# JiaruiFeng/KP-GNN

Hardware: AMD Instinct MI355X
Metric: graphs/sec KP-GIN fwd+bwd, ZINC-12k K=8 L=8 h=104 (higher is better)
Workload: dtype f32; 1 GPU; ZINC-12k-shaped synthetic molecules, KPGINPlus K=8 L=8 h=104 kernel=spd geometric combine, fwd+bwd+Adam, L1 loss; global_batch=2048, nodes_per_batch=47450, khop_edges_per_batch=1018372, active_pairs_per_batch=1018372, parallelism=dp1, launch=hipGraph replay of fwd+bwd, batches=4 pre-staged batches cycled

## Files before the change

kp_gnn_amd/csrc/wgrad.hip:

```cpp
#include <cstdlib>
#include <type_traits>

#include "bf3.h"
#include "kpgnn_common.h"

namespace kpgnn {
namespace {

constexpr int kWgradBlocks = 512;

struct WgParams {
    int64_t N; int O, I;
    const float* dy; int64_t dys;
    const float* x; int64_t xs;
    const float* xm; const float* xi; const float* xg; const float* xb; int xrelu;
    float* slab;
    int64_t slab_row, slab_off;
};
struct WgPair { WgParams q[2]; };

template <int TI, int RG>
__device__ __forceinline__ void wgrad_problem(const WgParams p, float* lds) {
    const int lane = threadIdx.x & 63;
    const int nstrip = (int)(blockDim.x >> 6) / RG;
    const int wave = (int)(threadIdx.x >> 6) % nstrip, rg = (int)(threadIdx.x >> 6) / nstrip;
    const int kk = lane >> 5, c = lane & 31;
    const int o = wave * 32 + c;
    const int64_t vgrid = (int64_t)gridDim.x * RG, vb = (int64_t)blockIdx.x * RG + rg;
    const bool o_ok = o < p.O;
    f32x16 acc[TI];
#pragma unroll
    for (int t = 0; t < TI; ++t)
        for (int v = 0; v < 16; ++v) acc[t][v] = 0.f;
    float bsum = 0.f;
    float tm[TI], ts[TI], tg[TI], tb[TI];
    const bool tr = p.xm != nullptr;
    if (tr) {
#pragma unroll
        for (int t = 0; t < TI; ++t) {
            const int i = t * 32 + c;
            const bool ok = i < p.I;
            tm[t] = ok ? p.xm[i] : 0.f; ts[t] = ok ? p.xi[i] : 0.f; tg[t] = ok ? p.xg[i] : 0.f; tb[t] = ok ? p.xb[i] : 0.f;
        }
    }
    const int64_t pairs = (p.N + 1) / 2;
    constexpr int UN = 4;
    const int dyo = kk * (int)p.dys + (o_ok ? o : p.O - 1);
    int xo[TI];
#pragma unroll
    for (int t = 0; t < TI; ++t) xo[t] = kk * (int)p.xs + min(t * 32 + c, p.I - 1);
    for (int64_t pr = vb; pr < pairs; pr += vgrid * UN) {
        float a[UN], b[UN][TI];
        const bool full = 2 * (pr + (int64_t)(UN - 1) * vgrid) + 1 < p.N;
        if (full) {
#pragma unroll
            for (int u = 0; u < UN; ++u) {
                const int64_t r0 = 2 * (pr + (int64_t)u * vgrid);
                const float* dyr = p.dy + r0 * p.dys;
                const float* xr = p.x + r0 * p.xs;
                a[u] = dyr[dyo];
#pragma unroll
                for (int t = 0; t < TI; ++t) b[u][t] = xr[xo[t]];
            }
            if (tr) {
#pragma unroll
                for (int u = 0; u < UN; ++u)
#pragma unroll
                    for (int t = 0; t < TI; ++t) {
                        float v = fmaf((b[u][t] - tm[t]) * ts[t], tg[t], tb[t]);
                        if (p.xrelu) v = fmaxf(v, 0.f);
                        b[u][t] = v;
                    }
            }
        } else {
#pragma unroll
            for (int u = 0; u < UN; ++u) {
                const int64_t r = 2 * (pr + (int64_t)u * vgrid) + kk;
                const bool r_ok = r < p.N;
                a[u] = (r_ok && o_ok) ? p.dy[r * p.dys + o] : 0.f;
#pragma unroll
                for (int t = 0; t < TI; ++t) {
                    const int i = t * 32 + c;
                    b[u][t] = (r_ok && i < p.I) ? p.x[r * p.xs + i] : 0.f;
                }
            }
            if (tr) {
#pragma unroll
                for (int u = 0; u < UN; ++u) {
                    const bool r_ok = 2 * (pr + (int64_t)u * vgrid) + kk < p.N;
#pragma unroll
                    for (int t = 0; t < TI; ++t) {
                        float v = fmaf((b[u][t] - tm[t]) * ts[t], tg[t], tb[t]);
                        if (p.xrelu) v = fmaxf(v, 0.f);
                        b[u][t] = (r_ok && t * 32 + c < p.I) ? v : 0.f;
                    }
                }
            }
        }
#pragma unroll
        for (int u = 0; u < UN; ++u) {
            bsum += a[u];
#pragma unroll
            for (int t = 0; t < TI; ++t) acc[t] = __builtin_amdgcn_mfma_f32_32x32x2f32(a[u], b[u][t], acc[t], 0, 0, 0);
        }
    }
    bsum += __shfl_xor(bsum, 32);
    if (RG > 1) {
        float* sl = lds + (size_t)wave * (TI * 16 + 1) * 64 + lane;
        __syncthreads();
        if (rg == 1) {
#pragma unroll
            for (int t = 0; t < TI; ++t)
                for (int v = 0; v < 16; ++v) sl[(t * 16 + v) * 64] = acc[t][v];
            sl[TI * 16 * 64] = bsum;
        }
        __syncthreads();
        if (rg == 0) {
#pragma unroll
            for (int t = 0; t < TI; ++t)
                for (int v = 0; v < 16; ++v) acc[t][v] += sl[(t * 16 + v) * 64];
            bsum += sl[TI * 16 * 64];
        }
    }
    float* out = p.slab + (int64_t)blockIdx.x * p.slab_row + p.slab_off;
    if (rg == 0) {
#pragma unroll
    for (int t = 0; t < TI; ++t) {
        const int i = t * 32 + c;
        for (int v = 0; v < 16; ++v) {
            const int orow = wave * 32 + (v & 3) + 8 * (v >> 2) + 4 * kk;
            if (orow < p.O && i < p.I) out[(int64_t)orow * p.I + i] = acc[t][v];
        }
    }
    if (kk == 0 && o_ok) out[(int64_t)p.O * p.I + o] = bsum;
    }
}

template <int TI, int RG>
__global__ void __launch_bounds__(512)
wgrad_kernel(const WgPair pp, int nprob) {
    extern __shared__ __attribute__((aligned(16))) float wg_lds[];
    if (gridDim.y > 1) {
        if (blockIdx.y == 0) wgrad_problem<TI, RG>(pp.q[0], wg_lds);
        else wgrad_problem<TI, RG>(pp.q[1], wg_lds);
        return;
    }
    wgrad_problem<TI, RG>(pp.q[0], wg_lds);
    if (nprob > 1) wgrad_problem<TI, RG>(pp.q[1], wg_lds);
}

int wgrad_grid(int64_t N) {
    int64_t g = (N + 15) / 16;
    if (g > kWgradBlocks) g = kWgradBlocks;
    return (int)(g < 1 ? 1 : g);
}

int wgrad_check(const kpgnn_wgrad_desc* d, const char* who) {
    KPGNN_REQUIRE(d != nullptr, "%s: NULL descriptor", who);
    KPGNN_REQUIRE(d->N >= 1 && d->O >= 1 && d->I >= 1, "%s: bad N=%lld O=%d I=%d", who, (long long)d->N, d->O, d->I);
    if (d->O > 256 || d->I > 256) return fail(KPGNN_ELIMIT, "%s: O=%d, I=%d exceed 256", who, d->O, d->I);
    KPGNN_REQUIRE(d->dy && d->x && d->dw && d->dy_stride >= d->O && d->x_stride >= d->I, "%s: bad pointers/strides", who);
    KPGNN_REQUIRE(!d->x_mean || (d->x_invstd && d->x_gamma && d->x_beta), "%s: x transform needs mean, invstd, gamma, beta", who);
    return KPGNN_OK;
}

WgParams wgrad_params(const kpgnn_wgrad_desc* d, float* slab, int64_t slab_row, int64_t slab_off) {
    WgParams p;
    p.N = d->N; p.O = d->O; p.I = d->I; p.dy = d->dy; p.dys = d->dy_stride; p.x = d->x; p.xs = d->x_stride;
    p.xm = d->x_mean; p.xi = d->x_invstd; p.xg = d->x_gamma; p.xb = d->x_beta; p.xrelu = d->x_relu;
    p.slab = slab; p.slab_row = slab_row; p.slab_off = slab_off;
    return p;
}

int wgrad_groups(int O) { return O <= 128 ? 2 : 1; }

int wgrad_blocks(int64_t N, int O) {
    const int rg = wgrad_groups(O);
    return (wgrad_grid(N) + rg - 1) / rg;
}

int wgrad_launch(const WgPair& pp, int nprob, int O, int I, int grid, hipStream_t s) {
    const int waves = (O + 31) / 32, ti = (I + 31) / 32, rg = wgrad_groups(O);
    dim3 blk(waves * 64 * rg), gr(grid, (nprob > 1 && grid * rg <= 128) ? 2 : 1);
    const size_t lds = rg > 1 ? sizeof(float) * (size_t)waves * (ti * 16 + 1) * 64 : 0;
#define KP_WG(T) do { \
        if (rg > 1) { KPGNN_HIP_TRY(ensure_dynamic_lds((const void*)wgrad_kernel<T, 2>, lds)); \
                      hipLaunchKernelGGL((wgrad_kernel<T, 2>), gr, blk, lds, s, pp, nprob); } \
        else hipLaunchKernelGGL((wgrad_kernel<T, 1>), gr, blk, 0, s, pp, nprob); } while (0)
    switch (ti) {
        case 1: KP_WG(1); break;
        case 2: KP_WG(2); break;
        case 3: KP_WG(3); break;
        case 4: KP_WG(4); break;
        case 5: KP_WG(5); break;
        case 6: KP_WG(6); break;
        case 7: KP_WG(7); break;
        default: KP_WG(8); break;
    }
#undef KP_WG
    KPGNN_LAUNCH_CHECK("wgrad_kernel");
    return KPGNN_OK;
}

constexpr int kW2Rows = 32;
constexpr int kW2MaxProb = 16;

struct Wg2Prob {
    const float* dy; const float* x; const float* mask;
    const float* xm; const float* xi; const float* xg; const float* xb;
    int xrelu;
    int64_t dys, xs, out_off, bias_off;
};
struct Wg2Args {
    int64_t N; const int32_t* n_dyn;
    int O, I, nprob; int64_t ldw;
    float* slab; int64_t slab_row;
    Wg2Prob q[kW2MaxProb];
};

template <int TI>
__global__ void __launch_bounds__(256, 2)
wgrad2_kernel(const Wg2Args A) {
    extern __shared__ __attribute__((aligned(16))) float w2[];
    constexpr int R = kW2Rows;
    const int O = A.O, I = A.I;
    float* dyl = w2;
    float* xl = w2 + R * O;
    float* coef = xl + R * I;
    const int tid = threadIdx.x, wave = tid >> 6, lane = tid & 63;
    const int kk = lane >> 5, c = lane & 31;
    const int nprob = A.nprob;
    const int pi = (int)(blockIdx.x % nprob), slice = (int)(blockIdx.x / nprob), nslices = (int)(gridDim.x / nprob);
    Wg2Prob q = A.q[0];
#pragma unroll
    for (int i = 1; i < kW2MaxProb; ++i)
        if (pi == i) q = A.q[i];
    const int64_t N = A.n_dyn ? (int64_t)min((int64_t)*A.n_dyn, A.N) : A.N;
    const bool tr = q.xm != nullptr;
    if (tr)
        for (int i = tid; i < I; i += 256) { coef[i] = q.xm[i]; coef[I + i] = q.xi[i]; coef[2 * I + i] = q.xg[i]; coef[3 * I + i] = q.xb[i]; }
    const int o4 = O >> 2, i4 = I >> 2;
    int dy_row[4], dy_cg[4], x_row[TI], x_cg[TI];
#pragma unroll
    for (int j = 0; j < 4; ++j) { const int e = tid + 256 * j; dy_row[j] = e < R * o4 ? e / o4 : -1; dy_cg[j] = e % o4; }
#pragma unroll
    for (int j = 0; j < TI; ++j) { const int e = tid + 256 * j; x_row[j] = e < R * i4 ? e / i4 : -1; x_cg[j] = e % i4; }
    float4 pdy[4], pm[4], px[TI];
    const bool has_mask = q.mask != nullptr;
    const int64_t last = N - 1;
    auto issue = [&](int64_t ch) {
        const int64_t r0 = ch * R;
#pragma unroll
        for (int j = 0; j < 4; ++j) {
            const int64_t r = min(r0 + max(dy_row[j], 0), last);
            pdy[j] = *reinterpret_cast<const float4*>(q.dy + r * q.dys + 4 * dy_cg[j]);
            if (has_mask) pm[j] = *reinterpret_cast<const float4*>(q.mask + r * q.dys + 4 * dy_cg[j]);
        }
#pragma unroll
        for (int j = 0; j < TI; ++j) {
            const int64_t r = min(r0 + max(x_row[j], 0), last);
            px[j] = *reinterpret_cast<const float4*>(q.x + r * q.xs + 4 * x_cg[j]);
        }
    };
    auto commit = [&](int64_t ch) {
        const int64_t r0 = ch * R;
        const float4 zero = make_float4(0.f, 0.f, 0.f, 0.f);
#pragma unroll
        for (int j = 0; j < 4; ++j) {
            float4 v = pdy[j];
            if (has_mask) { v.x = pm[j].x > 0.f ? v.x : 0.f; v.y = pm[j].y > 0.f ? v.y : 0.f; v.z = pm[j].z > 0.f ? v.z : 0.f; v.w = pm[j].w > 0.f ? v.w : 0.f; }
            if (r0 + dy_row[j] >= N) v = zero;
            if (dy_row[j] >= 0) *reinterpret_cast<float4*>(dyl + dy_row[j] * O + 4 * dy_cg[j]) = v;
        }
#pragma unroll
        for (int j = 0; j < TI; ++j) {
            float4 v = px[j];
            if (tr) {
                const float4 m = *reinterpret_cast<const float4*>(coef + 4 * x_cg[j]), s = *reinterpret_cast<const float4*>(coef + I + 4 * x_cg[j]);
                const float4 g = *reinterpret_cast<const float4*>(coef + 2 * I + 4 * x_cg[j]), b = *reinterpret_cast<const float4*>(coef + 3 * I + 4 * x_cg[j]);
                v.x = fmaf((v.x - m.x) * s.x, g.x, b.x); v.y = fmaf((v.y - m.y) * s.y, g.y, b.y);
                v.z = fmaf((v.z - m.z) * s.z, g.z, b.z); v.w = fmaf((v.w - m.w) * s.w, g.w, b.w);
                if (q.xrelu) { v.x = fmaxf(v.x, 0.f); v.y = fmaxf(v.y, 0.f); v.z = fmaxf(v.z, 0.f); v.w = fmaxf(v.w, 0.f); }
            }
            if (r0 + x_row[j] >= N) v = zero;
            if (x_row[j] >= 0) *reinterpret_cast<float4*>(xl + x_row[j] * I + 4 * x_cg[j]) = v;
        }
    };
    f32x16 acc[TI];
#pragma unroll
    for (int t = 0; t < TI; ++t)
        for (int v = 0; v < 16; ++v) acc[t][v] = 0.f;
    float bsum = 0.f;
    const int o = wave * 32 + c;
    const bool o_ok = o < O;
    const float* ap = dyl + kk * O + (o_ok ? o : O - 1);
    const float* bp[TI];
#pragma unroll
    for (int t = 0; t < TI; ++t) bp[t] = xl + kk * I + min(t * 32 + c, I - 1);
    const int64_t chunks = (N + R - 1) / R;
    int64_t ch = slice;
    if (tr) __syncthreads();
    if (ch < chunks) { issue(ch); commit(ch); }
    __syncthreads();
    for (; ch < chunks; ch += nslices) {
        const int64_t nx = ch + nslices;
        const bool more = nx < chunks;
        if (more) issue(nx);
#pragma unroll
        for (int p2 = 0; p2 < R / 2; ++p2) {
            const float a = ap[2 * p2 * O];
            bsum += a;
#pragma unroll
            for (int t = 0; t < TI; ++t) acc[t] = __builtin_amdgcn_mfma_f32_32x32x2f32(a, bp[t][2 * p2 * I], acc[t], 0, 0, 0);
        }
        __syncthreads();
        if (more) commit(nx);
        __syncthreads();
    }
    bsum += __shfl_xor(bsum, 32);
    float* out = A.slab + (int64_t)slice * A.slab_row;
#pragma unroll
    for (int t = 0; t < TI; ++t) {
        const int i = t * 32 + c;
        for (int v = 0; v < 16; ++v) {
            const int orow = wave * 32 + (v & 3) + 8 * (v >> 2) + 4 * kk;
            if (orow < O && i < I) out[q.out_off + (int64_t)orow * A.ldw + i] = acc[t][v];
        }
    }
    if (q.bias_off >= 0 && kk == 0 && o_ok) out[q.bias_off + o] = bsum;
}

constexpr int kW3Pitch = 40;

constexpr int kW3Blocks = 256;

template <int TI, bool MASK>
__global__ void __launch_bounds__(512, 1)
wgrad3_kernel(const Wg2Args A) {
    extern __shared__ __attribute__((aligned(16))) float w2[];
    constexpr int R = kW2Rows, P = kW3Pitch;
    const int O = A.O, I = A.I;
    const int bufsz = 3 * (O + I) * P;
    __bf16* pl = reinterpret_cast<__bf16*>(w2);
    float* coef = reinterpret_cast<float*>(pl + 2 * bufsz);
    const int tid = threadIdx.x, lane = tid & 63;
    const int wave = __builtin_amdgcn_readfirstlane(tid >> 6);
    const int kg = lane >> 5, c = lane & 31;
    const int nprob = A.nprob;
    const int pi = (int)(blockIdx.x % nprob), slice = (int)(blockIdx.x / nprob), nslices = (int)(gridDim.x / nprob);
    Wg2Prob q = A.q[0];
#pragma unroll
    for (int i = 1; i < kW2MaxProb; ++i)
        if (pi == i) q = A.q[i];
    const int64_t N = A.n_dyn ? (int64_t)min((int64_t)*A.n_dyn, A.N) : A.N;
    const bool tr = q.xm != nullptr;
    if (tr)
        for (int i = tid; i < I; i += 512) { coef[i] = q.xm[i]; coef[I + i] = q.xi[i]; coef[2 * I + i] = q.xg[i]; coef[3 * I + i] = q.xb[i]; }
    const int64_t chunks = (N + R - 1) / R;
    const int64_t mine = slice < chunks ? (chunks - slice + nslices - 1) / nslices : 0;
    const bool producer = wave >= 4;
    const bool is_x = wave >= 6;
    const int ncg = (is_x ? I : O) >> 2;
    const int task = tid & 127;
    const bool owner = producer && task < 4 * ncg;
    const int g = owner ? task & 3 : 0, cg = owner ? task >> 2 : 0;
    const float* src = is_x ? q.x : q.dy;
    const int64_t sstride = is_x ? q.xs : q.dys;
    const uint32_t sbytes = (uint32_t)sstride * 4u;
    const bool xform = tr && is_x;
    const int64_t last = N - 1;
    bf3_f2 bs01 = {0.f, 0.f}, bs23 = {0.f, 0.f};
    auto produce = [&](auto mask_c) {
        constexpr bool M = decltype(mask_c)::value;
        float4 pv0[8], pm0[8], pv1[8], pm1[8];
        auto issue = [&](int64_t k, float4 (&pv)[8], float4 (&pm)[8]) {
            const int64_t c0 = (slice + min(k, mine - 1) * nslices) * R;
            const float* cp = src + c0 * sstride;
            const float* mp = M ? q.mask + c0 * sstride : nullptr;
            const int lim = (int)min((int64_t)R, N - c0) - 1;
#pragma unroll
            for (int j = 0; j < 8; ++j) {
                const uint32_t off = __umul24((uint32_t)min(8 * g + j, lim), sbytes) + 16u * (uint32_t)cg;
                pv[j] = *reinterpret_cast<const float4*>(reinterpret_cast<const char*>(cp) + off);
                if (M) pm[j] = *reinterpret_cast<const float4*>(reinterpret_cast<const char*>(mp) + off);
            }
        };
        auto commit = [&](int64_t k, float4 (&pv)[8], float4 (&pm)[8]) {
            const int64_t c0 = (slice + min(k, mine - 1) * nslices) * R;
            if (M) {
    #pragma unroll
                for (int j = 0; j < 8; ++j) {
                    pv[j].x = pm[j].x > 0.f ? pv[j].x : 0.f; pv[j].y = pm[j].y > 0.f ? pv[j].y : 0.f;
                    pv[j].z = pm[j].z > 0.f ? pv[j].z : 0.f; pv[j].w = pm[j].w > 0.f ? pv[j].w : 0.f;
                }
            }
            if (xform) {
                const float4 m4 = *reinterpret_cast<const float4*>(coef + 4 * cg), s4 = *reinterpret_cast<const float4*>(coef + I + 4 * cg);
                const float4 g4 = *reinterpret_cast<const float4*>(coef + 2 * I + 4 * cg), b4 = *reinterpret_cast<const float4*>(coef + 3 * I + 4 * cg);
    #pragma unroll
                for (int j = 0; j < 8; ++j) {
                    float4 v = pv[j];
                    v.x = fmaf((v.x - m4.x) * s4.x, g4.x, b4.x); v.y = fmaf((v.y - m4.y) * s4.y, g4.y, b4.y);
                    v.z = fmaf((v.z - m4.z) * s4.z, g4.z, b4.z); v.w = fmaf((v.w - m4.w) * s4.w, g4.w, b4.w);
                    if (q.xrelu) { v.x = fmaxf(v.x, 0.f); v.y = fmaxf(v.y, 0.f); v.z = fmaxf(v.z, 0.f); v.w = fmaxf(v.w, 0.f); }
                    pv[j] = v;
                }
            }
            if (c0 + R > N) {
    #pragma unroll
                for (int j = 0; j < 8; ++j)
                    if (c0 + 8 * g + j >= N) pv[j] = make_float4(0.f, 0.f, 0.f, 0.f);
            }
            if (!is_x && k < mine) {
    #pragma unroll
                for (int j = 0; j < 8; ++j) { bs01 += bf3_f2{pv[j].x, pv[j].y}; bs23 += bf3_f2{pv[j].z, pv[j].w}; }
            }
            if (owner) {
                __bf16* base = pl + (k & 1) * bufsz + (is_x ? 3 * O * P : 0) + 8 * g;
                const int cols = is_x ? I : O;
    #pragma unroll
                for (int e2 = 0; e2 < 2; ++e2) {
                    bf3_u2 h[8], m[8], l[8];
#pragma unroll
                    for (int j = 0; j < 8; ++j)
                        bf3_split2(e2 == 0 ? bf3_f2{pv[j].x, pv[j].y} : bf3_f2{pv[j].z, pv[j].w}, h[j], m[j], l[j]);
                    __bf16* col = base + (4 * cg + 2 * e2) * P;
                    *reinterpret_cast<uint4*>(col) = make_uint4(bf3_pack(h[0].x, h[1].x), bf3_pack(h[2].x, h[3].x), bf3_pack(h[4].x, h[5].x), bf3_pack(h[6].x, h[7].x));
                    *reinterpret_cast<uint4*>(col + P) = make_uint4(bf3_pack(h[0].y, h[1].y), bf3_pack(h[2].y, h[3].y), bf3_pack(h[4].y, h[5].y), bf3_pack(h[6].y, h[7].y));
                    *reinterpret_cast<uint4*>(col + cols * P) = make_uint4(bf3_pack(m[0].x, m[1].x), bf3_pack(m[2].x, m[3].x), bf3_pack(m[4].x, m[5].x), bf3_pack(m[6].x, m[7].x));
                    *reinterpret_cast<uint4*>(col + cols * P + P) = make_uint4(bf3_pack(m[0].y, m[1].y), bf3_pack(m[2].y, m[3].y), bf3_pack(m[4].y, m[5].y), bf3_pack(m[6].y, m[7].y));
                    *reinterpret_cast<uint4*>(col + 2 * cols * P) = make_uint4(bf3_pack(l[0].x, l[1].x), bf3_pack(l[2].x, l[3].x), bf3_pack(l[4].x, l[5].x), bf3_pack(l[6].x, l[7].x));
                    *reinterpret_cast<uint4*>(col + 2 * cols * P + P) = make_uint4(bf3_pack(l[0].y, l[1].y), bf3_pack(l[2].y, l[3].y), bf3_pack(l[4].y, l[5].y), bf3_pack(l[6].y, l[7].y));
                }
            }
        };
        __builtin_amdgcn_s_setprio(2);
        if (mine > 0) {
            issue(0, pv0, pm0);
            issue(1, pv1, pm1);
            commit(0, pv0, pm0);
            issue(2, pv0, pm0);
        }
        __syncthreads();
        for (int64_t k = 0; k < mine; k += 2) {
            commit(k + 1, pv1, pm1);
            issue(k + 3, pv1, pm1);
            __syncthreads();
            commit(k + 2, pv0, pm0);
            issue(k + 4, pv0, pm0);
            __syncthreads();
        }
    };
    f32x16 acc[TI];
#pragma unroll
    for (int t = 0; t < TI; ++t)
        for (int v = 0; v < 16; ++v) acc[t][v] = 0.f;
    const int o = wave * 32 + c;
    const bool strip = !producer && wave * 32 < O;
    const int aoff = min(o, O - 1) * P + 8 * kg;
    int boff[TI];
#pragma unroll
    for (int t = 0; t < TI; ++t) boff[t] = 3 * O * P + min(t * 32 + c, I - 1) * P + 8 * kg;
    auto ld8 = [&](const __bf16* ptr) { return __builtin_bit_cast(bf3_x8, *reinterpret_cast<const uint4*>(ptr)); };
    auto multiply = [&](int64_t k) {
        const __bf16* bf = pl + (k & 1) * bufsz;
#pragma unroll
        for (int ks = 0; ks < R / 16; ++ks) {
            const bf3_x8 ah = ld8(bf + aoff + 16 * ks), am = ld8(bf + aoff + O * P + 16 * ks), al = ld8(bf + aoff + 2 * O * P + 16 * ks);
            bf3_x8 bh[TI], bm[TI], bl[TI];
#pragma unroll
            for (int t = 0; t < TI; ++t) {
                bh[t] = ld8(bf + boff[t] + 16 * ks); bm[t] = ld8(bf + boff[t] + I * P + 16 * ks); bl[t] = ld8(bf + boff[t] + 2 * I * P + 16 * ks);
            }
#pragma unroll
            for (int t = 0; t < TI; ++t) acc[t] = __builtin_amdgcn_mfma_f32_32x32x16_bf16(al, bh[t], acc[t], 0, 0, 0);
#pragma unroll
            for (int t = 0; t < TI; ++t) acc[t] = __builtin_amdgcn_mfma_f32_32x32x16_bf16(ah, bl[t], acc[t], 0, 0, 0);
#pragma unroll
            for (int t = 0; t < TI; ++t) acc[t] = __builtin_amdgcn_mfma_f32_32x32x16_bf16(am, bm[t], acc[t], 0, 0, 0);
#pragma unroll
            for (int t = 0; t < TI; ++t) acc[t] = __builtin_amdgcn_mfma_f32_32x32x16_bf16(am, bh[t], acc[t], 0, 0, 0);
#pragma unroll
            for (int t = 0; t < TI; ++t) acc[t] = __builtin_amdgcn_mfma_f32_32x32x16_bf16(ah, bm[t], acc[t], 0, 0, 0);
#pragma unroll
            for (int t = 0; t < TI; ++t) acc[t] = __builtin_amdgcn_mfma_f32_32x32x16_bf16(ah, bh[t], acc[t], 0, 0, 0);
        }
    };
    if (tr) __syncthreads();
    float* out = A.slab + (int64_t)slice * A.slab_row;
    if (producer) {
        if (MASK && !is_x) produce(std::true_type{});
        else produce(std::false_type{});
    } else {
        __syncthreads();
        for (int64_t k = 0; k < mine; k += 2) {
            if (strip) multiply(k);

            __syncthreads();

            if (strip && k + 1 < mine) multiply(k + 1);

            __syncthreads();
        }
        if (strip) {
#pragma unroll
            for (int t = 0; t < TI; ++t) {
                const int i = t * 32 + c;
                for (int v = 0; v < 16; ++v) {
                    const int orow = wave * 32 + (v & 3) + 8 * (v >> 2) + 4 * kg;
                    if (orow < O && i < I) out[q.out_off + (int64_t)orow * A.ldw + i] = acc[t][v];
                }
            }
        }
    }
    if (q.bias_off >= 0) {
        if (owner && !is_x) *reinterpret_cast<float4*>(coef + g * O + 4 * cg) = make_float4(bs01.x, bs01.y, bs23.x, bs23.y);
        __syncthreads();
        if (tid < O) out[q.bias_off + tid] = (coef[tid] + coef[O + tid]) + (coef[2 * O + tid] + coef[3 * O + tid]);
    }
}

bool wgrad3_ok(const Wg2Args& A) {
    for (int i = 1; i < A.nprob; ++i)
        if ((A.q[i].mask != nullptr) != (A.q[0].mask != nullptr)) return false;
    for (int i = 0; i < A.nprob; ++i)
        if (A.q[i].dys >= (1 << 22) || A.q[i].xs >= (1 << 22)) return false;
    return A.O <= 128 && A.I <= 128;
}
size_t wgrad3_lds(const Wg2Args& A) {
    const int m = A.O > A.I ? A.O : A.I;
    return (size_t)2 * 2 * 3 * (A.O + A.I) * kW3Pitch + sizeof(float) * 4 * (size_t)m;
}

bool wgrad2_ok(const kpgnn_wgrad_desc* d, const float* x) {
    auto al = [](const void* q) { return (((uintptr_t)q) & 15) == 0; };
    return d->O % 4 == 0 && d->I % 4 == 0 && d->O <= 128 && d->I <= 256 && d->dy_stride % 4 == 0 && d->x_stride % 4 == 0 &&
           al(d->dy) && al(x) && (!d->dy_mask || al(d->dy_mask));
}

Wg2Prob wgrad2_prob(const kpgnn_wgrad_desc* d, const float* x, int64_t out_off, int64_t bias_off) {
    Wg2Prob q;
    q.dy = d->dy; q.x = x; q.mask = d->dy_mask; q.xm = d->x_mean; q.xi = d->x_invstd; q.xg = d->x_gamma; q.xb = d->x_beta;
    q.xrelu = d->x_relu; q.dys = d->dy_stride; q.xs = d->x_stride; q.out_off = out_off; q.bias_off = bias_off;
    return q;
}

int wgrad2_slices(int64_t N, int nprob, int blocks) {
    const int64_t chunks = (N + kW2Rows - 1) / kW2Rows;
    int64_t s = blocks / nprob;
    if (s > chunks) s = chunks;
    return (int)(s < 1 ? 1 : s);
}

int wgrad2_launch(Wg2Args& A, int math, int* nslices, hipStream_t s) {
    const int ti = (A.I + 31) / 32;
    if (math != KPGNN_MATH_F32 && wgrad3_ok(A)) {
        *nslices = wgrad2_slices(A.N, A.nprob, kW3Blocks);
        dim3 gr3((unsigned)(*nslices * A.nprob)), blk3(512);
        const size_t lds3 = wgrad3_lds(A);
        const bool mask = A.q[0].mask != nullptr;
#define KP_W3(T) do { if (mask) { KPGNN_HIP_TRY(ensure_dynamic_lds((const void*)wgrad3_kernel<T, true>, lds3)); \
                                  hipLaunchKernelGGL((wgrad3_kernel<T, true>), gr3, blk3, lds3, s, A); } \
                      else { KPGNN_HIP_TRY(ensure_dynamic_lds((const void*)wgrad3_kernel<T, false>, lds3)); \
                             hipLaunchKernelGGL((wgrad3_kernel<T, false>), gr3, blk3, lds3, s, A); } } while (0)
        switch (ti) {
            case 1: KP_W3(1); break;
            case 2: KP_W3(2); break;
            case 3: KP_W3(3); break;
            default: KP_W3(4); break;
        }
#undef KP_W3
        KPGNN_LAUNCH_CHECK("wgrad3_kernel");
        return KPGNN_OK;
    }
    *nslices = wgrad2_slices(A.N, A.nprob, kWgradBlocks);
    dim3 gr((unsigned)(*nslices * A.nprob)), blk(256);
    const size_t lds = sizeof(float) * ((size_t)kW2Rows * (A.O + A.I) + 4 * (size_t)A.I);
#define KP_W2(T) hipLaunchKernelGGL((wgrad2_kernel<T>), gr, blk, lds, s, A)
    switch (ti) {
        case 1: KP_W2(1); break;
        case 2: KP_W2(2); break;
        case 3: KP_W2(3); break;
        case 4: KP_W2(4); break;
        case 5: KP_W2(5); break;
        case 6: KP_W2(6); break;
        case 7: KP_W2(7); break;
        default: KP_W2(8); break;
    }
#undef KP_W2
    KPGNN_LAUNCH_CHECK("wgrad2_kernel");
    return KPGNN_OK;
}

}
}

using namespace kpgnn;

extern "C" size_t kpgnn_wgrad_workspace_bytes(int32_t O, int32_t I) {
    if (O < 1 || I < 1) return 0;
    return sizeof(float) * ((size_t)kWgradBlocks * ((size_t)O * I + O) + O);
}

extern "C" int kpgnn_linear_wgrad(const kpgnn_wgrad_desc* d, kpgnn_stream_t stream) {
    int rc = wgrad_check(d, "linear_wgrad");
    if (rc != KPGNN_OK) return rc;
    KPGNN_REQUIRE(d->workspace && d->workspace_bytes >= kpgnn_wgrad_workspace_bytes(d->O, d->I), "linear_wgrad: workspace too small");
    const int64_t nw = (int64_t)d->O * d->I;
    float* slab = (float*)d->workspace;
    hipStream_t s = (hipStream_t)stream;
    int grid;
    if (wgrad2_ok(d, d->x)) {
        Wg2Args A;
        A.N = d->N; A.n_dyn = d->n_dyn; A.O = d->O; A.I = d->I; A.nprob = 1; A.ldw = d->I; A.slab = slab; A.slab_row = nw + d->O;
        for (int i = 0; i < kW2MaxProb; ++i) A.q[i] = wgrad2_prob(d, d->x, 0, nw);
        rc = wgrad2_launch(A, d->math, &grid, s);
    } else {
        KPGNN_REQUIRE(!d->dy_mask && !d->n_dyn, "linear_wgrad: dy_mask / n_dyn need 16-B aligned operands with O %% 4 == I %% 4 == 0, O <= 128");
        WgPair pp;
        pp.q[0] = pp.q[1] = wgrad_params(d, slab, nw + d->O, 0);
        grid = wgrad_blocks(d->N, d->O);
        rc = wgrad_launch(pp, 1, d->O, d->I, grid, s);
    }
    if (rc != KPGNN_OK) return rc;
    float* db = d->db ? d->db : slab + (size_t)kWgradBlocks * (nw + d->O);
    if (d->defer) {
        kpgnn_reduce_job* j = d->defer;
        j->slab = slab; j->nslab = grid; j->elems = nw + d->O;
        j->out[0] = d->dw; j->n_out[0] = nw; j->out[1] = db; j->n_out[1] = d->O;
        j->out[2] = j->out[3] = nullptr; j->n_out[2] = j->n_out[3] = 0;
        return KPGNN_OK;
    }
    return slab_reduce(slab, grid, nw + d->O, d->dw, nw, db, d->O, nullptr, s);
}

extern "C" int kpgnn_linear_wgrad_pair(const kpgnn_wgrad_desc* a, const kpgnn_wgrad_desc* b, kpgnn_stream_t stream) {
    int rc = wgrad_check(a, "linear_wgrad_pair");
    if (rc != KPGNN_OK) return rc;
    rc = wgrad_check(b, "linear_wgrad_pair");
    if (rc != KPGNN_OK) return rc;
    KPGNN_REQUIRE(a->O == b->O && a->I == b->I && a->N == b->N, "linear_wgrad_pair: the two problems must share N, O, I");
    KPGNN_REQUIRE(a->db && b->db, "linear_wgrad_pair: both bias gradients are required");
    KPGNN_REQUIRE(a->workspace && a->workspace_bytes >= 2 * kpgnn_wgrad_workspace_bytes(a->O, a->I), "linear_wgrad_pair: workspace too small");
    const int64_t nw = (int64_t)a->O * a->I, one = nw + a->O;
    float* slab = (float*)a->workspace;
    hipStream_t s = (hipStream_t)stream;
    int grid;
    if (wgrad2_ok(a, a->x) && wgrad2_ok(b, b->x)) {
        Wg2Args A;
        A.N = a->N; A.n_dyn = a->n_dyn; A.O = a->O; A.I = a->I; A.nprob = 2; A.ldw = a->I; A.slab = slab; A.slab_row = 2 * one;
        for (int i = 0; i < kW2MaxProb; ++i) A.q[i] = wgrad2_prob(a, a->x, 0, nw);
        A.q[1] = wgrad2_prob(b, b->x, one, one + nw);
        rc = wgrad2_launch(A, a->math, &grid, s);
    } else {
        KPGNN_REQUIRE(!a->dy_mask && !b->dy_mask && !a->n_dyn, "linear_wgrad_pair: dy_mask / n_dyn need 16-B aligned operands");
        WgPair pp;
        pp.q[0] = wgrad_params(a, slab, 2 * one, 0);
        pp.q[1] = wgrad_params(b, slab, 2 * one, one);
        grid = wgrad_blocks(a->N, a->O);
        rc = wgrad_launch(pp, 2, a->O, a->I, grid, s);
    }
    if (rc != KPGNN_OK) return rc;
    if (a->defer) {
        kpgnn_reduce_job* j = a->defer;
        j->slab = slab; j->nslab = grid; j->elems = 2 * one;
        j->out[0] = a->dw; j->n_out[0] = nw; j->out[1] = a->db; j->n_out[1] = a->O;
        j->out[2] = b->dw; j->n_out[2] = nw; j->out[3] = b->db; j->n_out[3] = b->O;
        return KPGNN_OK;
    }
    return slab_reduce(slab, grid, 2 * one, a->dw, nw, a->db, a->O, b->dw, s, nw, b->db);
}

extern "C" size_t kpgnn_wgrad_group_workspace_bytes(int32_t O, int32_t I, int32_t group) {
    if (O < 1 || I < 1 || group < 1 || group > kW2MaxProb) return 0;
    return sizeof(float) * ((size_t)(kWgradBlocks / group) * ((size_t)O * I * group + O) + O);
}

extern "C" int kpgnn_linear_wgrad_group(const kpgnn_wgrad_desc* d, const float* const* x_group, int32_t group, kpgnn_stream_t stream) {
    KPGNN_REQUIRE(d != nullptr && x_group != nullptr && group >= 1 && group <= kW2MaxProb, "linear_wgrad_group: bad arguments (1 <= group <= %d)", kW2MaxProb);
    kpgnn_wgrad_desc probe = *d;
    probe.x = x_group[0];
    int rc = wgrad_check(&probe, "linear_wgrad_group");
    if (rc != KPGNN_OK) return rc;
    for (int l = 0; l < group; ++l)
        if (!x_group[l] || !wgrad2_ok(d, x_group[l]))
            return fail(KPGNN_ELIMIT, "linear_wgrad_group: needs 16-B aligned operands, O %% 4 == I %% 4 == 0, O <= 128, I <= 256");
    KPGNN_REQUIRE(!d->x_mean, "linear_wgrad_group: no x transform");
    KPGNN_REQUIRE(d->workspace && d->workspace_bytes >= kpgnn_wgrad_group_workspace_bytes(d->O, d->I, group), "linear_wgrad_group: workspace too small");
    const int64_t nw = (int64_t)d->O * d->I * group;
    Wg2Args A;
    A.N = d->N; A.n_dyn = d->n_dyn; A.O = d->O; A.I = d->I; A.nprob = group; A.ldw = (int64_t)d->I * group;
    A.slab = (float*)d->workspace; A.slab_row = nw + d->O;
    for (int i = 0; i < kW2MaxProb; ++i) A.q[i] = wgrad2_prob(d, x_group[i < group ? i : 0], (int64_t)(i < group ? i : 0) * d->I, i == 0 ? nw : -1);
    int grid = 0;
    hipStream_t s = (hipStream_t)stream;
    rc = wgrad2_launch(A, d->math, &grid, s);
    if (rc != KPGNN_OK) return rc;
    float* db = d->db ? d->db : A.slab + (size_t)grid * A.slab_row;
    if (d->defer) {
        kpgnn_reduce_job* j = d->defer;
        j->slab = A.slab; j->nslab = grid; j->elems = nw + d->O;
        j->out[0] = d->dw; j->n_out[0] = nw; j->out[1] = db; j->n_out[1] = d->O;
        j->out[2] = j->out[3] = nullptr; j->n_out[2] = j->n_out[3] = 0;
        return KPGNN_OK;
    }
    return slab_reduce(A.slab, grid, nw + d->O, d->dw, nw, db, d->O, nullptr, s);
}
```

Measured before the change: 678,600 graphs/s.

## Handle ragged wgrad3 edge tiles with 16x16 MFMA and interleave producer waves

The bf16x3 weight-gradient kernel now plans its tiles so that any output or input remainder of at most 16 (e.g. h=104 = 3*32+8) is covered by 16x16x32 MFMA edge tiles, instead of padding to a full 32-wide strip. The template instantiation follows the count of full 32-column input tiles, and extra waves compute the row and column edge tiles alongside the main strips. Producer and consumer waves are interleaved across SIMDs rather than split into halves, and the producer priority boost is removed. This is meant to cut wasted MFMA work on padded tiles and balance the SIMDs, at the cost of more registers and more complex index logic.

```diff
diff --git a/kp_gnn_amd/csrc/wgrad.hip b/kp_gnn_amd/csrc/wgrad.hip
--- a/kp_gnn_amd/csrc/wgrad.hip
+++ b/kp_gnn_amd/csrc/wgrad.hip
@@ -211,10 +211,12 @@
     int xrelu;
     int64_t dys, xs, out_off, bias_off;
 };
+struct W3Plan { int nbo, nbi, eo, ei; };
 struct Wg2Args {
     int64_t N; const int32_t* n_dyn;
     int O, I, nprob; int64_t ldw;
     float* slab; int64_t slab_row;
+    W3Plan plan;
     Wg2Prob q[kW2MaxProb];
 };
 
@@ -331,6 +333,7 @@
 }
 
 constexpr int kW3Pitch = 40;
+using f32x4 = __attribute__((ext_vector_type(4))) float;
 
 constexpr int kW3Blocks = 256;
 
@@ -358,10 +361,11 @@
         for (int i = tid; i < I; i += 512) { coef[i] = q.xm[i]; coef[I + i] = q.xi[i]; coef[2 * I + i] = q.xg[i]; coef[3 * I + i] = q.xb[i]; }
     const int64_t chunks = (N + R - 1) / R;
     const int64_t mine = slice < chunks ? (chunks - slice + nslices - 1) / nslices : 0;
-    const bool producer = wave >= 4;
-    const bool is_x = wave >= 6;
+    const bool producer = (wave & 2) != 0;
+    const int ridx = (wave & 1) | ((wave >> 2) << 1);
+    const bool is_x = ridx >= 2;
     const int ncg = (is_x ? I : O) >> 2;
-    const int task = tid & 127;
+    const int task = (ridx & 1) * 64 + lane;
     const bool owner = producer && task < 4 * ncg;
     const int g = owner ? task & 3 : 0, cg = owner ? task >> 2 : 0;
     const float* src = is_x ? q.x : q.dy;
@@ -434,7 +438,6 @@
                 }
             }
         };
-        __builtin_amdgcn_s_setprio(2);
         if (mine > 0) {
             issue(0, pv0, pm0);
             issue(1, pv1, pm1);
@@ -451,23 +454,64 @@
             __syncthreads();
         }
     };
-    f32x16 acc[TI];
-#pragma unroll
-    for (int t = 0; t < TI; ++t)
+    constexpr int TB = TI > 0 ? TI : 1, NB = TI < 4 ? 2 * TI + 1 : 8, NR = TI < 4 ? 6 : 1;
+    const int nbo = A.plan.nbo;
+    const bool strip = !producer && ridx < nbo;
+    const bool edges = !producer && (nbo == 4 || ridx == 3);
+    const int nb = edges && A.plan.eo ? 2 * TI + (A.plan.ei ? 1 : 0) : 0;
+    const int nr = TI < 4 && edges && A.plan.ei ? (nbo == 4 ? 2 : 2 * nbo) : 0;
+    const int r0 = nbo == 4 ? 2 * ridx : 0;
+    const bool work = strip || nb > 0 || nr > 0;
+    f32x16 acc[TB];
+    f32x4 sb[NB], sr[NR];
+#pragma unroll
+    for (int t = 0; t < TB; ++t)
         for (int v = 0; v < 16; ++v) acc[t][v] = 0.f;
-    const int o = wave * 32 + c;
-    const bool strip = !producer && wave * 32 < O;
+#pragma unroll
+    for (int j = 0; j < NB; ++j) sb[j] = f32x4{0.f, 0.f, 0.f, 0.f};
+#pragma unroll
+    for (int j = 0; j < NR; ++j) sr[j] = f32x4{0.f, 0.f, 0.f, 0.f};
+    const int o = ridx * 32 + c;
     const int aoff = min(o, O - 1) * P + 8 * kg;
-    int boff[TI];
-#pragma unroll
-    for (int t = 0; t < TI; ++t) boff[t] = 3 * O * P + min(t * 32 + c, I - 1) * P + 8 * kg;
+    int boff[TB];
+#pragma unroll
+    for (int t = 0; t < TB; ++t) boff[t] = 3 * O * P + min(t * 32 + c, I - 1) * P + 8 * kg;
+    const int c16 = lane & 15, kq = lane >> 4;
+    const int sbA = min(32 * nbo + c16, O - 1) * P + 8 * kq;
+    const int srB = 3 * O * P + min(32 * TI + c16, I - 1) * P + 8 * kq;
+    int sbo[NB], sro[NR];
+#pragma unroll
+    for (int j = 0; j < NB; ++j) sbo[j] = 3 * O * P + min(16 * j + c16, I - 1) * P + 8 * kq;
+#pragma unroll
+    for (int j = 0; j < NR; ++j) sro[j] = min(16 * (r0 + j) + c16, O - 1) * P + 8 * kq;
     auto ld8 = [&](const __bf16* ptr) { return __builtin_bit_cast(bf3_x8, *reinterpret_cast<const uint4*>(ptr)); };
+    auto mma6s = [&](f32x4& d, const bf3_x8& ah, const bf3_x8& am, const bf3_x8& al, const bf3_x8& bh, const bf3_x8& bm, const bf3_x8& bl) {
+        d = __builtin_amdgcn_mfma_f32_16x16x32_bf16(al, bh, d, 0, 0, 0);
+        d = __builtin_amdgcn_mfma_f32_16x16x32_bf16(ah, bl, d, 0, 0, 0);
+        d = __builtin_amdgcn_mfma_f32_16x16x32_bf16(am, bm, d, 0, 0, 0);
+        d = __builtin_amdgcn_mfma_f32_16x16x32_bf16(am, bh, d, 0, 0, 0);
+        d = __builtin_amdgcn_mfma_f32_16x16x32_bf16(ah, bm, d, 0, 0, 0);
+        d = __builtin_amdgcn_mfma_f32_16x16x32_bf16(ah, bh, d, 0, 0, 0);
+    };
     auto multiply = [&](int64_t k) {
         const __bf16* bf = pl + (k & 1) * bufsz;
+        if (nb > 0) {
+            const bf3_x8 ah = ld8(bf + sbA), am = ld8(bf + sbA + O * P), al = ld8(bf + sbA + 2 * O * P);
+#pragma unroll
+            for (int j = 0; j < NB; ++j)
+                if (j < nb) mma6s(sb[j], ah, am, al, ld8(bf + sbo[j]), ld8(bf + sbo[j] + I * P), ld8(bf + sbo[j] + 2 * I * P));
+        }
+        if (nr > 0) {
+            const bf3_x8 bh = ld8(bf + srB), bm = ld8(bf + srB + I * P), bl = ld8(bf + srB + 2 * I * P);
+#pragma unroll
+            for (int j = 0; j < NR; ++j)
+                if (j < nr) mma6s(sr[j], ld8(bf + sro[j]), ld8(bf + sro[j] + O * P), ld8(bf + sro[j] + 2 * O * P), bh, bm, bl);
+        }
+        if (TI == 0 || !strip) return;
 #pragma unroll
         for (int ks = 0; ks < R / 16; ++ks) {
             const bf3_x8 ah = ld8(bf + aoff + 16 * ks), am = ld8(bf + aoff + O * P + 16 * ks), al = ld8(bf + aoff + 2 * O * P + 16 * ks);
-            bf3_x8 bh[TI], bm[TI], bl[TI];
+            bf3_x8 bh[TB], bm[TB], bl[TB];
 #pragma unroll
             for (int t = 0; t < TI; ++t) {
                 bh[t] = ld8(bf + boff[t] + 16 * ks); bm[t] = ld8(bf + boff[t] + I * P + 16 * ks); bl[t] = ld8(bf + boff[t] + 2 * I * P + 16 * ks);
@@ -494,11 +538,11 @@
     } else {
         __syncthreads();
         for (int64_t k = 0; k < mine; k += 2) {
-            if (strip) multiply(k);
+            if (work) multiply(k);
 
             __syncthreads();
 
-            if (strip && k + 1 < mine) multiply(k + 1);
+            if (work && k + 1 < mine) multiply(k + 1);
 
             __syncthreads();
         }
@@ -507,9 +551,25 @@
             for (int t = 0; t < TI; ++t) {
                 const int i = t * 32 + c;
                 for (int v = 0; v < 16; ++v) {
-                    const int orow = wave * 32 + (v & 3) + 8 * (v >> 2) + 4 * kg;
+                    const int orow = ridx * 32 + (v & 3) + 8 * (v >> 2) + 4 * kg;
                     if (orow < O && i < I) out[q.out_off + (int64_t)orow * A.ldw + i] = acc[t][v];
                 }
+            }
+        }
+#pragma unroll
+        for (int j = 0; j < NB; ++j) {
+            const int i = 16 * j + c16;
+            for (int v = 0; v < 4; ++v) {
+                const int orow = 32 * nbo + 4 * kq + v;
+                if (j < nb && orow < O && i < I) out[q.out_off + (int64_t)orow * A.ldw + i] = sb[j][v];
+            }
+        }
+#pragma unroll
+        for (int j = 0; j < NR; ++j) {
+            const int i = 32 * TI + c16;
+            for (int v = 0; v < 4; ++v) {
+                const int orow = 16 * (r0 + j) + 4 * kq + v;
+                if (j < nr && orow < O && i < I) out[q.out_off + (int64_t)orow * A.ldw + i] = sr[j][v];
             }
         }
     }
@@ -527,6 +587,12 @@
         if (A.q[i].dys >= (1 << 22) || A.q[i].xs >= (1 << 22)) return false;
     return A.O <= 128 && A.I <= 128;
 }
+W3Plan wgrad3_plan(int O, int I) {
+    W3Plan p;
+    p.eo = O % 32 <= 16 ? O % 32 : 0; p.ei = I % 32 <= 16 ? I % 32 : 0;
+    p.nbo = (O - p.eo + 31) / 32; p.nbi = (I - p.ei + 31) / 32;
+    return p;
+}
 size_t wgrad3_lds(const Wg2Args& A) {
     const int m = A.O > A.I ? A.O : A.I;
     return (size_t)2 * 2 * 3 * (A.O + A.I) * kW3Pitch + sizeof(float) * 4 * (size_t)m;
@@ -555,6 +621,7 @@
 int wgrad2_launch(Wg2Args& A, int math, int* nslices, hipStream_t s) {
     const int ti = (A.I + 31) / 32;
     if (math != KPGNN_MATH_F32 && wgrad3_ok(A)) {
+        A.plan = wgrad3_plan(A.O, A.I);
         *nslices = wgrad2_slices(A.N, A.nprob, kW3Blocks);
         dim3 gr3((unsigned)(*nslices * A.nprob)), blk3(512);
         const size_t lds3 = wgrad3_lds(A);
@@ -563,7 +630,8 @@
                                   hipLaunchKernelGGL((wgrad3_kernel<T, true>), gr3, blk3, lds3, s, A); } \
                       else { KPGNN_HIP_TRY(ensure_dynamic_lds((const void*)wgrad3_kernel<T, false>, lds3)); \
                              hipLaunchKernelGGL((wgrad3_kernel<T, false>), gr3, blk3, lds3, s, A); } } while (0)
-        switch (ti) {
+        switch (A.plan.nbi) {
+            case 0: KP_W3(0); break;
             case 1: KP_W3(1); break;
             case 2: KP_W3(2); break;
             case 3: KP_W3(3); break;
```

After: 682,300 graphs/s (median of 5 runs). Within noise of the previous version (+0.5%).
